# titus-leistner/mmlf

Hardware: AMD Instinct MI355X
Metric: 96x96 EPI patches/sec fwd+bwd, bs=512 (higher is better)
Workload: dtype f32 via 2 x f16 operand split (22 significant bits per operand, locally scaled; 3 MFMA passes, f32 accumulate)

## Files before the change

### mmlf_amd/csrc/wgrad.hip

```cpp
#include "conv_device.h"
#include "wgrad_map.h"

#ifdef MMLF_BOUNDS_DEBUG
int mmlf_oob_counts_wgrad(unsigned long long *host8, int reset)
{
    if (hipMemcpyFromSymbol(host8, HIP_SYMBOL(g_mmlf_oob), sizeof(unsigned long long) * 8) != hipSuccess) return 1;
    if (reset) {
        const unsigned long long z[8] = {};
        if (hipMemcpyToSymbol(HIP_SYMBOL(g_mmlf_oob), z, sizeof(z)) != hipSuccess) return 1;
    }
    return 0;
}
#endif

struct WgradArgs {
    const float *in;
    const float *g;
    float *part;
    long long NQpad;
    int cs_in, cin, cs_g, g_shift, P, nsplit, nslice, chunks_per_split, nchunks;
    int items;
    int g_cols;
    const float *in_amax, *g_amax;
    const float *chunk_scales;
// ... 150 lines not shown
__device__ __forceinline__ void split_store4(float4 v, char *p0, int plane_stride_bytes)
{
    unsigned h0, m0, l0, h1, m1, l1;
    split3_pair(v.x, v.y, h0, m0, l0);
    split3_pair(v.z, v.w, h1, m1, l1);
    *reinterpret_cast<uint2 *>(p0) = make_uint2(h0, h1);
    *reinterpret_cast<uint2 *>(p0 + plane_stride_bytes) = make_uint2(m0, m1);
    *reinterpret_cast<uint2 *>(p0 + 2 * plane_stride_bytes) = make_uint2(l0, l1);
}

template <int PL>
__device__ __forceinline__ void split_store4_pl(float4 v, float scale, char *p0, int plane_stride_bytes)
{
    if constexpr (PL == 3) {
        split_store4(v, p0, plane_stride_bytes);
    } else {
        unsigned h0, l0, h1, l1;
        split2_pair_f16<true>(v.x, v.y, scale, h0, l0);
        split2_pair_f16<true>(v.z, v.w, scale, h1, l1);
        *reinterpret_cast<uint2 *>(p0) = make_uint2(h0, h1);
        *reinterpret_cast<uint2 *>(p0 + plane_stride_bytes) = make_uint2(l0, l1);
    }
}
template <int PL>
__device__ __forceinline__ f32x4 mfma16_pl(bf16x8 x, bf16x8 y, f32x4 c)
{
    if constexpr (PL == 3) return __builtin_amdgcn_mfma_f32_16x16x32_bf16(x, y, c, 0, 0, 0);
    else return __builtin_amdgcn_mfma_f32_16x16x32_f16(__builtin_bit_cast(f16x8, x), __builtin_bit_cast(f16x8, y), c, 0, 0, 0);
}
template <int PL> __device__ __forceinline__ constexpr int term_a(int t)
{
    return PL == 3 ? (t == 0 ? 2 : t == 1 ? 0 : t <= 3 ? 1 : 0) : (t == 0 ? 1 : 0);
}
template <int PL> __device__ __forceinline__ constexpr int term_b(int t)
{
    return PL == 3 ? (t == 0 ? 0 : t == 1 ? 2 : t == 2 ? 1 : t == 3 ? 0 : t == 4 ? 1 : 0) : (t == 1 ? 1 : 0);
}
struct WgradScales { float inv_sa, inv_sg; };
template <int PL> __device__ __forceinline__ WgradScales wgrad_scales(const WgradArgs &a)
{
    WgradScales s = {1.f, 1.f};
    if constexpr (PL == 2) {
        s.inv_sa = a.chunk_scales[2 * (size_t)a.nchunks];
        s.inv_sg = a.chunk_scales[2 * (size_t)a.nchunks + 1];
    }
    return s;
}
template <int PL> __device__ __forceinline__ void wgrad_chunk_scale(const WgradArgs &a, int c, float &sa, float &sg)
{
    if constexpr (PL == 2) {
        const float2 v = *reinterpret_cast<const float2 *>(a.chunk_scales + 2 * (size_t)c);
        sa = __uint_as_float(__builtin_amdgcn_readfirstlane(__float_as_uint(v.x)));
        sg = __uint_as_float(__builtin_amdgcn_readfirstlane(__float_as_uint(v.y)));
    } else {
        sa = 1.f; sg = 1.f;
    }
}
struct ChunkScaleArgs {
    const float *in_amax, *g_amax;
    float *out;
    long long NQ;
    int nchunks, P, g_shift, nrows;
    Magic divP;
};
__device__ __forceinline__ int pow2_exponent(float p) { return (int)(__float_as_uint(p) >> 23) - 127; }
__global__ __launch_bounds__(256) void wgrad_chunk_scales_kernel(ChunkScaleArgs a)
{
    const int c = blockIdx.x * 256 + threadIdx.x;
    const float sA = pow2_scale_for(mmlf_amax_tensor_max(a.in_amax)), sG = pow2_scale_for(mmlf_amax_tensor_max(a.g_amax));
    if (c == 0) {
        a.out[2 * (size_t)a.nchunks] = 1.f / sA;
        a.out[2 * (size_t)a.nchunks + 1] = 1.f / sG;
    }
    if (c >= a.nchunks) return;
    const long long q0 = (long long)c * WG_KQ;
    int x = 0;
    if (q0 < a.NQ) {
        const long long ql = q0 + WG_KQ - 1;
        const unsigned r0 = fastdiv((unsigned)q0, a.divP);
        unsigned r1 = fastdiv((unsigned)(ql + a.P + 1), a.divP);
        if (r1 >= (unsigned)a.nrows) r1 = a.nrows - 1;
        float ma = 0.f, mg = 0.f;
        for (unsigned r = r0; r <= r1; ++r) ma = fmaxf(ma, a.in_amax[MMLF_AMAX_HEAD + r]);
        const unsigned g0 = fastdiv((unsigned)(q0 + a.g_shift), a.divP);
        unsigned g1 = fastdiv((unsigned)(ql + a.g_shift), a.divP);
        if (g1 >= (unsigned)a.nrows) g1 = a.nrows - 1;
        for (unsigned r = g0; r <= g1; ++r) mg = fmaxf(mg, a.g_amax[MMLF_AMAX_HEAD + r]);
        const int u = ma > 0.f ? pow2_exponent(pow2_scale_for(ma)) - pow2_exponent(sA) : 60;
        const int v = mg > 0.f ? pow2_exponent(pow2_scale_for(mg)) - pow2_exponent(sG) : 60;
        const int uu = u < 0 ? 0 : u, vv = v < 0 ? 0 : v;
        x = (uu - vv) >> 1;
        x = x > 15 ? 15 : (x < -24 ? -24 : x);
    }
    a.out[2 * (size_t)c] = sA * exp2f((float)x);
    a.out[2 * (size_t)c + 1] = sG * exp2f((float)-x);
}

template <int MB, int NB, int PL>
__global__ __launch_bounds__(256, 2) void wgrad4tap_x6n_kernel(WgradArgs a)
{
    constexpr int ROWA = 32 * (MB | 1), ROWG = 32 * (NB | 1);
    constexpr int A_PLANE = 34 * ROWA;
    constexpr int A_BYTES = 2 * PL * A_PLANE;
    constexpr int NTERM = PL == 3 ? 6 : 3;
    const WgradScales sc = wgrad_scales<PL>(a);
    constexpr int G_PLANE = WG_KQ * ROWG;
    constexpr int FA = 4 * MB, FG = 4 * NB;
    constexpr int NA = (66 * FA + 255) / 256, NG = (WG_KQ * FG + 255) / 256;
    constexpr bool HOLD_G = NB <= 5;
    extern __shared__ __attribute__((aligned(16))) char smem[];
    char *As = smem;
    char *Gs = smem + A_BYTES;

    const int tid = threadIdx.x;
    const int lane = tid & 63, t = tid >> 6;
    const int r16 = lane & 15, q4 = lane >> 4;
    int slice, split;
    if (!wgrad_block_map(blockIdx.x, a.nslice, a.nsplit, slice, split)) return;
    const int ci0 = slice * 16 * MB;
    int c_begin = split * a.chunks_per_split;
    int c_end = c_begin + a.chunks_per_split;
    if (c_end > a.nchunks) c_end = a.nchunks;

    f32x4 acc[MB][NB];
#pragma unroll
    for (int mb = 0; mb < MB; ++mb)
#pragma unroll
        for (int nb = 0; nb < NB; ++nb)
#pragma unroll
            for (int r = 0; r < 4; ++r) acc[mb][nb][r] = 0.f;

    float4 ra[NA], rg[NG];
#define WN_GLOAD(c)                                                                                         \
    do {                                                                                                    \
        const long long Qc = (long long)(c) * WG_KQ;                                                        \
        _Pragma("unroll") for (int j = 0; j < NA; ++j) {                                                    \
            const int idx = min(tid + 256 * j, 66 * FA - 1);                                                \
            const int row = idx / FA, f = idx - row * FA;                                                   \
            const int seg = row >= 33, pix = row - 33 * seg;                                                \
            const int ch = min(ci0 + 4 * f, a.cs_in - 4);                                                   \
            MMLF_OOB(OOB_WG_IN, ((Qc + seg * a.P + pix) * a.cs_in + ch + 4) * 4ll > a.in_bytes);            \
            ra[j] = *reinterpret_cast<const float4 *>(a.in + (size_t)(Qc + seg * a.P + pix) * a.cs_in + ch); \
        }                                                                                                   \
        _Pragma("unroll") for (int j = 0; j < NG; ++j) {                                                    \
            const int idx = min(tid + 256 * j, WG_KQ * FG - 1);                                             \
            const int row = idx / FG, f = idx - row * FG;                                                   \
            const int gc = min(4 * f, a.g_cols - 4);                                                        \
            MMLF_OOB(OOB_WG_G, ((Qc + a.g_shift + row) * a.cs_g + gc + 4) * 4ll > a.g_bytes);               \
            rg[j] = *reinterpret_cast<const float4 *>(a.g + (size_t)(Qc + a.g_shift + row) * a.cs_g + gc);  \
        }                                                                                                   \
    } while (0)
#define WN_LSTORE()                                                                                         \
    do {                                                                                                    \
        _Pragma("unroll") for (int j = 0; j < NA; ++j) {                                                    \
            const int idx = min(tid + 256 * j, 66 * FA - 1);                                                \
            const int row = idx / FA, f = idx - row * FA;                                                   \
            const int seg = row >= 33, pix = row - 33 * seg;                                                \
            float4 v = ra[j];                \
            const int ch = ci0 + 4 * f;      \
            if (ch == a.cin) v.x = sc.inv_sa;                                        \
            if (ch + 1 == a.cin) v.y = sc.inv_sa;                                                           \
            if (ch + 2 == a.cin) v.z = sc.inv_sa;                                                           \
            if (ch + 3 == a.cin) v.w = sc.inv_sa;                                                           \
            split_store4_pl<PL>(v, st_sa, As + seg * PL * A_PLANE + pix * ROWA + 8 * f, A_PLANE);           \
        }                                                                                                   \
        _Pragma("unroll") for (int j = 0; j < NG; ++j) {                                                    \
            const int idx = min(tid + 256 * j, WG_KQ * FG - 1);                                             \
            const int row = idx / FG, f = idx - row * FG;                                                   \
            split_store4_pl<PL>(rg[j], st_sg, Gs + row * ROWG + 8 * f, G_PLANE);                            \
        }                                                                                                   \
    } while (0)
    const int tq = (lane & 15) >> 2, tp = lane & 3;
    const char *a_lane = As + (t >> 1) * PL * A_PLANE + ((t & 1) + 4 * q4 + tq) * ROWA + 8 * tp;
    const char *g_lane = Gs + (4 * q4 + tq) * ROWG + 8 * tp;

    float st_sa = 1.f, st_sg = 1.f;
    if (c_begin < c_end) {
        WN_GLOAD(c_begin);
        for (int c = c_begin; c < c_end; ++c) {
            wgrad_chunk_scale<PL>(a, c, st_sa, st_sg);
            WN_LSTORE();
            __syncthreads();
            if (c + 1 < c_end) WN_GLOAD(c + 1);
            if constexpr (HOLD_G) {
                bf16x8 gf[NB][PL];
#pragma unroll
                for (int nb = 0; nb < NB; ++nb)
#pragma unroll
                    for (int pl = 0; pl < PL; ++pl) gf[nb][pl] = tr_frag(g_lane + pl * G_PLANE + 32 * nb, 4 * ROWG);
#pragma unroll
                for (int mb = 0; mb < MB; ++mb) {
                    bf16x8 af[PL];
#pragma unroll
                    for (int pl = 0; pl < PL; ++pl) af[pl] = tr_frag(a_lane + pl * A_PLANE + 32 * mb, 4 * ROWA);
#pragma unroll
                    for (int term = 0; term < NTERM; ++term)
#pragma unroll
                        for (int nb = 0; nb < NB; ++nb)
                            acc[mb][nb] = mfma16_pl<PL>(af[term_a<PL>(term)], gf[nb][term_b<PL>(term)], acc[mb][nb]);
                }
            } else {
                bf16x8 af[MB][PL];
#pragma unroll
                for (int mb = 0; mb < MB; ++mb)
#pragma unroll
                    for (int pl = 0; pl < PL; ++pl) af[mb][pl] = tr_frag(a_lane + pl * A_PLANE + 32 * mb, 4 * ROWA);
#pragma unroll
                for (int nb = 0; nb < NB; ++nb) {
                    bf16x8 gf[PL];
#pragma unroll
                    for (int pl = 0; pl < PL; ++pl) gf[pl] = tr_frag(g_lane + pl * G_PLANE + 32 * nb, 4 * ROWG);
#pragma unroll
                    for (int term = 0; term < NTERM; ++term)
#pragma unroll
                        for (int mb = 0; mb < MB; ++mb)
                            acc[mb][nb] = mfma16_pl<PL>(af[mb][term_a<PL>(term)], gf[term_b<PL>(term)], acc[mb][nb]);
                }
            }
            __syncthreads();
        }
    }
#undef WN_GLOAD
#undef WN_LSTORE
    constexpr int NP = 16 * NB;
    const int CIP = a.nslice * 16 * MB;
    float *pp = a.part + ((size_t)(split * 4 + t) * CIP + ci0) * NP;
#pragma unroll
    for (int mb = 0; mb < MB; ++mb)
#pragma unroll
        for (int nb = 0; nb < NB; ++nb)
#pragma unroll
            for (int r = 0; r < 4; ++r) {
                const int row = 16 * mb + 4 * q4 + r;
                const float un = (ci0 + row == a.cin ? 1.f : sc.inv_sa) * sc.inv_sg;
                MMLF_OOB(OOB_WG_PART, (long long)(pp - a.part) + (long long)row * NP + 16 * nb + r16 >= a.part_floats);
                pp[(size_t)row * NP + 16 * nb + r16] = acc[mb][nb][r] * un;
            }
}

template <int MB, int NBH, int PL>
__global__ __launch_bounds__(512, 2) void wgrad4tap_x6w_kernel(WgradArgs a)
{
    constexpr int NB = 2 * NBH;
    const WgradScales sc = wgrad_scales<PL>(a);
    constexpr int ROWA = 32 * (MB | 1), ROWG = 32 * (NB | 1);
    constexpr int A_PLANE = 34 * ROWA;
    constexpr int A_BYTES = 2 * PL * A_PLANE;
    constexpr int G_PLANE = WG_KQ * ROWG;
    constexpr int BUF_BYTES = A_BYTES + PL * G_PLANE;
    constexpr int FA = 4 * MB, FG = 4 * NB;
    constexpr int NA = (66 * FA + 511) / 512, NG = (WG_KQ * FG + 511) / 512;
    static_assert(2 * BUF_BYTES <= 160 * 1024, "LDS");
    extern __shared__ __attribute__((aligned(16))) char smem[];

    const int tid = threadIdx.x;
    const int lane = tid & 63;
    const int w = __builtin_amdgcn_readfirstlane(tid >> 6);
    const int t = w & 3, h = w >> 2;
    const int q4 = lane >> 4;

    float4 ra[NA], rg[NG];

    unsigned ga_off[NA], gg_off[NG];
    int la_off[NA], lg_off[NG], a_ch[NA];
#pragma unroll
    for (int j = 0; j < NA; ++j) {
        const int idx = min(tid + 512 * j, 66 * FA - 1);
        const int row = idx / FA, f = idx - row * FA;
        const int seg = row >= 33, pix = row - 33 * seg;
        la_off[j] = seg * PL * A_PLANE + pix * ROWA + 8 * f;
    }
#pragma unroll
    for (int j = 0; j < NG; ++j) {
        const int idx = min(tid + 512 * j, WG_KQ * FG - 1);
        const int row = idx / FG, f = idx - row * FG;
        gg_off[j] = (unsigned)((a.g_shift + row) * a.cs_g + min(4 * f, a.g_cols - 4)) * 4u;
        lg_off[j] = A_BYTES + row * ROWG + 8 * f;
    }
    const char *const in_b = reinterpret_cast<const char *>(a.in), *const g_b = reinterpret_cast<const char *>(a.g);
#define WW_GLOAD_A(j, c)                                                                                    \
    do {                                                                                                    \
        const long long cb_ = (long long)(c) * WG_KQ * a.cs_in * 4;                         \
        MMLF_OOB(OOB_WG_IN, cb_ + ga_off[j] + 16 > a.in_bytes);                                             \
         \
         \
        const __amdgpu_buffer_rsrc_t rs_ = __builtin_amdgcn_make_buffer_rsrc(                               \
            const_cast<char *>(in_b + cb_), 0, mmlf_records_left(a.in_bytes, cb_), MMLF_BUF_FLAGS);         \
        ra[j] = __builtin_bit_cast(float4, __builtin_amdgcn_raw_buffer_load_b128(rs_, ga_off[j], 0, 0));    \
    } while (0)
#define WW_GLOAD_G(j, c)                                                                                    \
// ... 187 lines not shown
    constexpr int U = 16;
    double acc[U];
#pragma unroll
    for (int u = 0; u < U; ++u) acc[u] = 0.0;
    int sp = 0;
    for (; sp + U <= nsplit; sp += U) {
        float v[U];
#pragma unroll
        for (int u = 0; u < U; ++u) v[u] = pp[(size_t)(sp + u) * stride];
#pragma unroll
        for (int u = 0; u < U; ++u) acc[u] += v[u];
    }
    for (; sp < nsplit; ++sp) acc[0] += pp[(size_t)sp * stride];
#pragma unroll
    for (int h = U / 2; h > 0; h >>= 1)
#pragma unroll
        for (int u = 0; u < h; ++u) acc[u] += acc[u + h];
    const double s = acc[0];
    if (ci == Cin) {
        gb[co] = accumulate ? gb[co] + (float)s : (float)s;
    } else {
        const size_t o = ((size_t)co * Cin + ci) * NTAP + master_tap<(NTAP == 4 ? 2 : 3)>(t, variant);
        gw[o] = accumulate ? gw[o] + (float)s : (float)s;
    }
}

__global__ __launch_bounds__(256) void wgrad_reduce_wave_kernel(const float *__restrict__ part, float *__restrict__ gw,
                                                                float *__restrict__ gb, int Cin, int Cout, int CIP, int NP,
                                                                int nsplit, int variant, int accumulate)
{
    const int total = 4 * (Cin + 1) * Cout;
    const int idx = blockIdx.x * 4 + (threadIdx.x >> 6), lane = threadIdx.x & 63;
    if (idx >= total) return;
    const int co = idx % Cout;
    int r = idx / Cout;
    const int ci = r % (Cin + 1);
    const int t = r / (Cin + 1);
    if (ci == Cin && (t != 0 || gb == nullptr)) return;
    const float *pp = part + ((size_t)t * CIP + ci) * NP + co;
    const size_t stride = (size_t)4 * CIP * NP;
    double acc = 0.0;
    for (int sp = lane; sp < nsplit; sp += 64) acc += pp[(size_t)sp * stride];
#pragma unroll
    for (int o = 32; o > 0; o >>= 1) acc += __shfl_xor(acc, o);
    if (lane) return;
    if (ci == Cin) {
        gb[co] = accumulate ? gb[co] + (float)acc : (float)acc;
    } else {
        const size_t o = ((size_t)co * Cin + ci) * 4 + master_tap<2>(t, variant);
        gw[o] = accumulate ? gw[o] + (float)acc : (float)acc;
    }
}

static int wgrad_nsplit(int nslice)
{
    int n = 512 / nslice;
    n = n / 8 * 8;
    if (n < 8) n = 8;
    return n;
}

struct Wgrad16Cfg { int mb, nb, nslice, nsplit; };
static inline bool wgrad16_cfg(int Cin, int Cout, long long nchunks, Wgrad16Cfg *c)
{
    if (Cout <= 0 || Cout > 288) return false;
    c->nb = Cout <= 32 ? 2 : Cout <= 80 ? 5 : Cout <= 128 ? 8 : 18;
    if (c->nb == 18) {
        c->mb = 3;
        wgrad_wide_splits(Cin, nchunks, device_cus(), c->nslice, c->nsplit);
    } else {
        c->mb = (c->nb <= 5 && Cin + 1 > 32 && Cin + 1 <= 80) ? 5 : 2;
        if (c->nb == 8 && Cin + 1 >= 128) c->mb = 3;
        c->nslice = (Cin + 1 + 16 * c->mb - 1) / (16 * c->mb);
        c->nsplit = wgrad_nsplit(c->nslice);
    }
    return true;
}

constexpr int WGRAD_MAX_COUT = 288, WGRAD_MAX_COUT_WIDE = 512;
static inline int wgrad_col_blocks(int Cout) { return Cout > WGRAD_MAX_COUT ? 2 : 1; }
static inline int wgrad_block_cout(int Cout, int b) { return b == 0 ? (Cout < WGRAD_MAX_COUT ? Cout : WGRAD_MAX_COUT) : Cout - WGRAD_MAX_COUT; }

struct WgradBlock {
    int c0, cout;
    int nt;
    Wgrad16Cfg cfg;
    int nslice, nsplit;
    int CIP, NP;
    int64_t part_floats;
};
struct WgradPlan {
    int nblocks;
    WgradBlock blk[2];
    int64_t part_floats;
    int64_t scales_off;
};
static bool wgrad_f32_block(int ks, int Cin, int c0, int cout, WgradBlock &k)
{
    k = {};
    k.c0 = c0; k.cout = cout; k.nt = pick_nt(cout);
    if (k.nt < 0) return false;
    const int ci_slices = (Cin + 1 + 31) / 32;
    k.nslice = (ks == 2 ? WgradF32Shape<2>::BPS : WgradF32Shape<3>::BPS) * ci_slices;
    k.nsplit = wgrad_nsplit(k.nslice);
    k.CIP = ci_slices * 32; k.NP = k.nt * 32;
    k.part_floats = (int64_t)k.nsplit * ks * ks * k.CIP * k.NP;
    return true;
}
static void wgrad_split_block(const Wgrad16Cfg &c, WgradBlock &k)
{
    k.nt = 0; k.cfg = c; k.nslice = c.nslice; k.nsplit = c.nsplit;
    k.CIP = c.nslice * 16 * c.mb; k.NP = 16 * c.nb;
    k.part_floats = (int64_t)k.nsplit * 4 * k.CIP * k.NP;
}
static bool wgrad_plan(int planes, int Cin, int Cout, long long nchunks, WgradPlan &p)
{
    p = {};
    if (Cout > WGRAD_MAX_COUT_WIDE) return false;
    p.nblocks = wgrad_col_blocks(Cout);
    for (int b = 0, c0 = 0; b < p.nblocks; c0 += p.blk[b++].cout) {
        WgradBlock &k = p.blk[b];
        WgradBlock largest = {};
        Wgrad16Cfg c;
        if (!wgrad_f32_block(2, Cin, c0, wgrad_block_cout(Cout, b), k)) return false;
        int64_t sized = k.part_floats;
        if (wgrad16_cfg(Cin, k.cout, -1, &c)) {
            wgrad_split_block(c, largest);
            if (largest.part_floats > sized) sized = largest.part_floats;
        }
        sized = (sized + 3) / 4 * 4;
        if (sized > p.scales_off) p.scales_off = sized;
        if (planes && wgrad16_cfg(Cin, k.cout, nchunks, &c)) wgrad_split_block(c, k);
        if (k.part_floats > p.part_floats) p.part_floats = k.part_floats;
    }
    return true;
}

extern "C" int64_t mmlf_wgrad_workspace_floats(int Cin, int Cout, int B, int H, int W)
{
    WgradPlan p;
    if (!wgrad_plan(0, Cin, Cout, -1, p) || B <= 0 || H <= 0 || W <= 0) return -1;
    return p.scales_off + 2 * (make_grid(B, H, W).NQpad / WG_KQ) + 4;
}

template <int KS, int NT>
static int launch_wgrad_f32(const WgradArgs &a, hipStream_t st)
{
    using S = WgradF32Shape<KS>;
    const dim3 grid(wgrad_grid_blocks(a.nslice, a.nsplit)), block(64 * S::WAVES);
    if constexpr (KS == 2) hipLaunchKernelGGL(wgrad4tap_kernel<NT>, grid, block, S::lds_bytes(NT), st, a);
    else hipLaunchKernelGGL(wgrad9tap_kernel<NT>, grid, block, S::lds_bytes(NT), st, a);
    return mmlf_launch_status(KS == 2 ? "mmlf_conv2x2_wgrad" : "mmlf_conv3x3_wgrad");
}

template <int MB, int NB, int PL>
static int launch_wgrad16(const WgradArgs &a, hipStream_t st)
{
    constexpr size_t lds = 2 * PL * 34 * 32 * (MB | 1) + PL * WG_KQ * 32 * (NB | 1);
    static PerDeviceOnce attr_once;
    if (attr_once.run([] { return mmlf_allow_lds(reinterpret_cast<const void *>(wgrad4tap_x6n_kernel<MB, NB, PL>), lds, "mmlf_conv2x2_wgrad_split"); }))
        return 1;
    hipLaunchKernelGGL((wgrad4tap_x6n_kernel<MB, NB, PL>), dim3(wgrad_grid_blocks(a.nslice, a.nsplit)), dim3(256), lds, st, a);
    return mmlf_launch_status("mmlf_conv2x2_wgrad_split");
}

static bool wgrad_persist()
{
    static const bool on = [] { const char *e = getenv("MMLF_WGRAD_PERSIST"); return !e || atoi(e) != 0; }();
    return on;
}

template <int PL>
static int launch_wgrad_wide(const WgradArgs &a, hipStream_t st)
{
    constexpr size_t lds = 2 * (2 * PL * 34 * 32 * (3 | 1) + PL * WG_KQ * 32 * (18 | 1));
    static PerDeviceOnce attr_once;
    if (attr_once.run([] { return mmlf_allow_lds(reinterpret_cast<const void *>(wgrad4tap_x6w_kernel<3, 9, PL>), lds, "mmlf_conv2x2_wgrad_split(wide)"); }))
        return 1;
    hipLaunchKernelGGL((wgrad4tap_x6w_kernel<3, 9, PL>), dim3(wgrad_wide_grid(a.items, device_cus(), wgrad_persist())), dim3(512), lds, st, a);
    return mmlf_launch_status("mmlf_conv2x2_wgrad_split");
}

template <int PL>
static int launch_wgrad_split(const Wgrad16Cfg &c, const WgradArgs &a, hipStream_t st)
{
    switch (10 * c.mb + c.nb) {
    case 22: return launch_wgrad16<2, 2, PL>(a, st);
    case 52: return launch_wgrad16<5, 2, PL>(a, st);
    case 25: return launch_wgrad16<2, 5, PL>(a, st);
    case 55: return launch_wgrad16<5, 5, PL>(a, st);
    case 28: return launch_wgrad16<2, 8, PL>(a, st);
    case 38: return launch_wgrad16<3, 8, PL>(a, st);
    default: return launch_wgrad_wide<PL>(a, st);
    }
}

static WgradArgs wgrad_args(const float *in, int cs_in, int Cin, const float *g, int cs_g, int g_shift, float *workspace,
                            const Grid &gr, long long alloc, long long part_floats)
{
    WgradArgs a = {};
    a.in = in; a.g = g; a.part = workspace; a.NQpad = gr.NQpad;
    a.cs_in = cs_in; a.cin = Cin; a.cs_g = a.g_cols = cs_g; a.g_shift = g_shift; a.P = gr.P;
    a.in_bytes = alloc * cs_in * 4; a.g_bytes = alloc * cs_g * 4;
    a.part_floats = part_floats;
    a.nchunks = (int)(gr.NQpad / WG_KQ);
    return a;
}
static void wgrad_set_grid(WgradArgs &a, int nslice, int nsplit)
{
    a.nslice = nslice;
    a.nsplit = nsplit;
    a.chunks_per_split = (a.nchunks + nsplit - 1) / nsplit;
    a.items = (int)wgrad_grid_blocks(nslice, nsplit);
}

template <int KS>
static int wgrad_reduce(const WgradArgs &a, float *gw, float *gb, int Cin, int Cout, int CIP, int NP, int variant,
                        int accumulate, hipStream_t st)
{
    const int total = KS * KS * (Cin + 1) * Cout;
    hipLaunchKernelGGL(wgrad_reduce_kernel<KS * KS>, dim3((total + 255) / 256), dim3(256), 0, st, a.part, gw, gb, Cin, Cout,
                       CIP, NP, a.nsplit, variant, accumulate);
// ... 252 lines not shown
```

### mmlf_amd/csrc/wgrad_map.h

```cpp
#pragma once

__host__ __device__ __forceinline__ bool wgrad_block_map(int b, int nslice, int nsplit, int &slice, int &split)
{
    const int x = b & 7, j = b >> 3;
    const int reg = (nsplit >> 3) * nslice;
    if (j < reg) {
        slice = j % nslice;
        split = (j / nslice) * 8 + x;
        return true;
    }
    const int left = (nsplit & 7) * nslice, per = (left + 7) >> 3;
    const int m = x * per + (j - reg);
    slice = m % nslice;
    split = (nsplit & ~7) + m / nslice;
    return m < left;
}

static inline unsigned wgrad_grid_blocks(int nslice, int nsplit)
{
    return 8u * (unsigned)((nsplit >> 3) * nslice + ((nsplit & 7) * nslice + 7) / 8);
}

static inline void wgrad_wide_splits(int Cin, long long nchunks, int cus, int &nslice, int &nsplit)
{
    nslice = (Cin + 1 + 47) / 48;
    if (cus > 256 || nchunks < 0) cus = 256;
    const int one_round = cus / nslice, three_rounds = (768 / nslice + 7) / 8 * 8;
    nsplit = nchunks < 0 ? (one_round > three_rounds ? one_round : three_rounds)
                         : (nchunks >= 42 * 1024 ? three_rounds : one_round);
    if (nsplit < 8) nsplit = 8;
}

static inline unsigned wgrad_wide_grid(int items, int cus, bool persist)
{
    if (!persist) return (unsigned)items;
    int resident = cus / 8 * 8;
    if (resident < 8) resident = 8;
    return (unsigned)(items < resident ? items : resident);
}
```

### mmlf_amd/engine.py

```python
import ctypes
import os
import threading

import torch

from . import _lib
from ._lib import call, check, ptr

VAR_IDENTITY, VAR_TRANSPOSE, VAR_TRANSPOSE_FLIPH = 0, 1, 2
BN_BLOCKS = 1024
LOSS_BLOCKS = 1024


MAX_WIDTH = {2: 512, 3: 288}
MAX_OC = 288
MAX_OVERLAP_WIDTH = 288


def cs_of(c):
    return (c + 7) // 8 * 8


class Geometry:

# ... 138 lines not shown
CONV_MODE = os.environ.get('MMLF_CONV_MODE', 'f16x3')
_PACK = {'f16x3': ('mmlf_packed_filter_h2_bytes', 1, 'mmlf_pack_filter_h2'),
         'bf16x6': ('mmlf_packed_filter_split_bytes', 1, 'mmlf_pack_filter_split'),
         'f32': ('mmlf_packed_filter_floats', 4, 'mmlf_pack_filter')}
_PACK3 = ('mmlf_packed_filter3x3_floats', 4, 'mmlf_pack_filter3x3')


def _pack(who, query, unit, entry, w, variant, dgrad):
    cout, cin = w.shape[0], w.shape[1]
    K, N = (cout, cin) if dgrad else (cin, cout)
    n = int(getattr(_lib.load(), query)(cs_of(K), N))
    if n < 0:
        raise RuntimeError(f'{who}: unsupported channels K={K} N={N}')
    out = torch.empty(n * unit // 4, dtype=torch.float32, device=w.device)
    call(entry, ptr(w), ptr(out), cout, cin, variant, int(dgrad), _lib.stream_ptr())
    return out


def pack_filter(w, variant, dgrad):
    return _pack('pack_filter', *_PACK.get(CONV_MODE, _PACK['f32']), w, variant, dgrad)


PROFILE = None


def _tic():
    e0, e1 = torch.cuda.Event(enable_timing=True), torch.cuda.Event(enable_timing=True)
    e0.record()
    return e0, e1


def _toc(events, tag, flops, nbytes):
    events[1].record()
    PROFILE.append((tag, flops, events[0], events[1], nbytes))


def _amax_of(geo, t, cs):
    a = getattr(t, 'absmax', None)
    if a is None:
        return geo.amax_of(t, cs)
    if CHECK_ABSMAX:
        true = geo.amax_of(t, cs)
        c = geo.amax_canonical(a)
        exact = geo.P >= 32
        bad = (c != true) if exact else (c < true)
        bad[0] = c[0] != true[0]
        if bool(bad.any()):
            k = int(bad.nonzero()[0])
            raise AssertionError(f'amax entry {k} holds {float(c[k])!r}, true max |x| is {float(true[k])!r}')
    return a


CHECK_ABSMAX = bool(os.environ.get('MMLF_CHECK_ABSMAX'))
OVERLAP_WGRAD = os.environ.get('MMLF_OVERLAP_WGRAD', '1') not in ('', '0')


CHECK_EXTENTS = bool(os.environ.get('MMLF_CHECK_EXTENTS'))
EXTENT_CHECKS = 0


def _audit(entry, scalars, n_ends, kind, have):
    global EXTENT_CHECKS
    ends = (ctypes.c_int64 * n_ends)()
    call(entry, *scalars, ends)
    for name, (k, t, off) in have.items():
        if t is None:
            continue
        got = t.untyped_storage().nbytes() - t.storage_offset() * t.element_size() - 4 * off
        if ends[k] > got:
            raise RuntimeError(f'MMLF_CHECK_EXTENTS: {kind}: the launch may touch {ends[k]} bytes behind `{name}`, '
                               f'the tensor has {got}')
    EXTENT_CHECKS += 1


def relu_bwd_slice(geo, src, cs_src, c_off, ref, cs_ref, ref_off, C, dst, cs_dst):
    amax = getattr(dst, 'absmax', None)
    if CHECK_EXTENTS:
        _audit('mmlf_audit_relu_bwd_slice', (cs_src, c_off, cs_ref, ref_off, C, cs_dst, geo.B, geo.H, geo.W), 4,
               f'relu_bwd_slice C={C} {cs_src}+{c_off} B={geo.B} {geo.H}x{geo.W}',
               {'src': (0, src, 0), 'ref': (1, ref, 0), 'dst': (2, dst, 0), 'amax': (3, amax, 0)})
    call('mmlf_relu_bwd_slice', ptr(src), cs_src, c_off, ptr(ref), cs_ref, ref_off, C, ptr(dst), cs_dst, geo.B, geo.H, geo.W,
         ptr(amax), _lib.stream_ptr())


THIN_MAX_N, THIN_MIN_K = 2, 64


def wgrad(geo, x, cs_in, cin, g, cs_g, cout, g_shift, gw, gb, variant, workspace, side=False):
    if cout <= THIN_MAX_N and cin >= THIN_MIN_K and cs_in <= 512:
        ws = _Workspace.get(x.device).scratch('thin_wgrad_side' if side else 'thin_wgrad', int(_lib.load().mmlf_conv2x2_wgrad_thin_workspace_floats(cin)))
        call('mmlf_conv2x2_wgrad_thin', ptr(x), cs_in, cin, ptr(g), cs_g, cout, g_shift, ptr(gw), ptr(gb), variant, 1,
             ptr(ws), geo.B, geo.H, geo.W, _lib.stream_ptr())
        return
    args = (ptr(x), cs_in, cin, ptr(g), cs_g, cout, g_shift, ptr(gw), ptr(gb), variant, 1, ptr(workspace),
            geo.B, geo.H, geo.W)
    prof = PROFILE is not None and cin >= 256 and cout >= 256
    if prof:
        events = _tic()
    if CONV_MODE == 'f16x3':
        ax, ag = _amax_of(geo, x, cs_in), _amax_of(geo, g, cs_g)
        if CHECK_EXTENTS:
            _audit('mmlf_audit_wgrad_h2', (cs_in, cin, cs_g, cout, g_shift, geo.B, geo.H, geo.W), 7,
                   f'wgrad {cin}->{cout} B={geo.B} {geo.H}x{geo.W} g_shift={g_shift}',
                   {'in': (0, x, 0), 'g': (1, g, 0), 'gw': (2, gw, 0), 'gb': (3, gb, 0), 'workspace': (4, workspace, 0),
                    'in_amax': (5, ax, 0), 'g_amax': (6, ag, 0)})
        call('mmlf_conv2x2_wgrad_h2', *args, ptr(ax), ptr(ag), _lib.stream_ptr())
    else:
# ... 291 lines not shown
            dev = stacks[0].device
            for name, t in zip('hvid', stacks):
                check(t, f'{name}_views', dev, shape=shape)
        self.check_params(p, dev)
        if packed is None:
            geo = Geometry(B, H, W, self.ksize)
        _Workspace.get(dev).enter_stream()
        fold = self.batchnorm and not train and (not save or (bool(frozen) and self.ksize == 2))
        relu_only = not self.batchnorm or fold
        packs = self._prepack(p, dev, save, input_grads, fold)
        tracked = []
        tape = {'geo': geo, 'device': dev, 'streams': [], 'out': [], 'packs': packs}
        if packed is not None:
            concat, xs = geo.buf(4 * self.chs, dev), list(xs_in)
        else:
            concat, *xs = geo.bufs([4 * self.chs] + [cs_of(cin0)] * 3, dev)
            xs.append(geo.buf(cs_of(cin0), dev))
        deferred = [] if (not fold and self.chs % 2 == 0 and all(b[-1].bn for _, _, b in self.streams)) else None
        for s, (key, var, blocks) in enumerate(self.streams):
            x = xs[s]
            if packed is None:
                call('mmlf_pack_nchw', ptr(stacks[s]), cin0, ptr(x), cs_of(cin0), B, H, W, ptr(x.absmax), _lib.stream_ptr())
            cs_x = cs_of(cin0)
            recs = []
            x_relu, xmask = False, None
            for k, spec in enumerate(blocks):
                last = k == len(blocks) - 1
                x, cs_x, xmask = self._block_fwd(geo, spec, var, x, cs_x, x_relu, xmask, p, train, recs if save else None,
                                                 out=concat if last else None, cs_out=4 * self.chs, c_off=s * self.chs,
                                                 packs=packs, tracked=tracked, deferred=deferred if last else None, fold=fold)
                x_relu = relu_only
            tape['streams'].append(recs)
        if deferred:
            arr = lambda k: (ctypes.c_void_p * 4)(*[ptr(d[k]) for d in deferred])
            call('mmlf_bn_apply_relu4', arr(0), cs_of(self.chs), self.chs, arr(1), arr(2), ptr(concat), 4 * self.chs,
                 B, H, W, ptr(concat.absmax), _lib.stream_ptr())
            del deferred[:]
        if save and relu_only:
            tape['concat'] = concat
        x, cs_x, x_relu, xmask = concat, 4 * self.chs, False, None
        for spec in self.out_blocks:
            x, cs_x, xmask = self._block_fwd(geo, spec, VAR_IDENTITY, x, cs_x, x_relu, xmask, p, train,
                                             tape['out'] if save else None, packs=packs, tracked=tracked, fold=fold)
            x_relu = relu_only
        if tracked:
            counts = {}
            for t in tracked:
                counts.setdefault(t.data_ptr(), [t, 0])[1] += 1
            torch._foreach_add_([t for t, _ in counts.values()], [n for _, n in counts.values()])
        out = torch.empty((B, self.oc, H, W), dtype=torch.float32, device=dev)
        call('mmlf_unpack_nchw', ptr(x), cs_x, ptr(out), self.oc, B, H, W, _lib.stream_ptr())
        return out, (tape if save else None)

    def _block_bwd(self, geo, rec, p, grads, gy, cs_gy, c_off, need_dx, after_bn=None, overlap=False, packs=None):
        spec, var = rec.spec, rec.var
        dev = gy.device
        ws = _Workspace.get(dev)
        B, H, W = geo.B, geo.H, geo.W
        C, cs_mid = spec.cout, cs_of(spec.cout)
        x, cs_x, y, z = rec.x, rec.cs_x, rec.y, rec.z
        pre = spec.prefix
        sp = _lib.stream_ptr
        packs = packs or {}
        f16 = CONV_MODE == 'f16x3' and self.ksize == 2
        bn = rec.bn
        assert grads is None or rec.pk2d is None, 'a frozen forward (BatchNorm folded) has no parameter gradients'
        if grads is not None:
            gw1, gb1, gw2, gb2 = (grads[f'{pre}.{k}'] for k in ('0.weight', '0.bias', '2.weight', '2.bias'))

        y_relu = {'mask_in': rec.ymask} if rec.ymask is not None and f16 else {'ref': y, 'cs_ref': cs_mid}
        x_relu = {}
        if rec.x_relu:
            x_relu = {'mask_in': rec.xmask} if rec.xmask is not None and f16 else {'ref': x, 'cs_ref': cs_x}

        got = geo.bufs(([cs_mid] if bn else []) + [cs_mid] + ([cs_x] if need_dx else []), dev)
        dy = got[1 if bn else 0]
        dx = got[-1] if need_dx else None
        if bn:
            if grads is None and rec.eval:
                coef = torch.zeros(3 * C, dtype=torch.float32, device=dev)
                coef[:C].copy_(rec.scale)
            else:
                coef = torch.empty(3 * C, dtype=torch.float32, device=dev)
                if grads is None:
                    dgb = ws.scratch('bn_dgamma_dbeta', 2 * C)
                    dgamma, dbeta, acc = dgb[:C], dgb[C:2 * C], 0
                else:
                    dgamma, dbeta, acc = grads[f'{pre}.3.weight'], grads[f'{pre}.3.bias'], 1
                call('mmlf_bn_bwd_reduce', ptr(gy), cs_gy, c_off, ptr(z), cs_mid, C, ptr(rec.scale), ptr(rec.shift),
                     ptr(p[f'{pre}.3.weight']), ptr(rec.smean), ptr(rec.sinv), ptr(dgamma), ptr(dbeta), acc, ptr(coef),
                     ptr(ws.partial), BN_BLOCKS, B, H, W, sp())
                if rec.eval:
                    coef[C:].zero_()
            dz = got[0]
            call('mmlf_bn_bwd_apply', ptr(gy), cs_gy, c_off, ptr(z), cs_mid, C, ptr(rec.scale), ptr(rec.shift),
                 ptr(rec.smean), ptr(coef), ptr(dz), cs_mid, B, H, W, ptr(dz.absmax), sp())
        else:
            assert c_off == 0 and cs_gy == cs_mid
            dz = gy
        if after_bn:
            after_bn()
        if grads is not None:
            self._wgrad(geo, True, y, cs_mid, C, dz, cs_mid, C, gw2, gb2, var)
        pk2d = rec.pk2d if rec.pk2d is not None else self._packed(packs, p, f'{pre}.2.weight', var, True)
        self._dgrad(geo, True, dz, cs_mid, C, pk2d, C, dy, cs_mid, **y_relu)
        del dz, got
        if overlap and need_dx and grads is not None:
            self._dgrad(geo, False, dy, cs_mid, C, self._packed(packs, p, f'{pre}.0.weight', var, True), spec.cin, dx, cs_x,
                        **x_relu)
            main = torch.cuda.current_stream()
            ready = main.record_event()
            with torch.cuda.stream(ws.side):
                ws.side.wait_event(ready)
                self._wgrad(geo, False, x, cs_x, spec.cin, dy, cs_mid, C, gw1, gb1, var, side=True)
                done = ws.side.record_event()
            return dx, done, (x, dy)
        if grads is not None:
            self._wgrad(geo, False, x, cs_x, spec.cin, dy, cs_mid, C, gw1, gb1, var)
        if need_dx:
            self._dgrad(geo, False, dy, cs_mid, C, self._packed(packs, p, f'{pre}.0.weight', var, True), spec.cin, dx, cs_x,
                        **x_relu)
        return dx, None, None

    def backward(self, p, tape, grad_output, grads, on_done=None, input_grads=None):
        geo, dev = tape['geo'], tape['device']
        check(grad_output, 'grad_output', dev, shape=(geo.B, self.oc, geo.H, geo.W), contiguous=False)
        if grads is not None:
            self._check_dict('grads', grads, self._grad_names, dev)
        _Workspace.get(dev).enter_stream()
        B, H, W = geo.B, geo.H, geo.W
        cs = cs_of(self.oc)
        g = geo.buf(cs, dev)
        call('mmlf_pack_nchw', ptr(grad_output.contiguous()), self.oc, ptr(g), cs, B, H, W, ptr(g.absmax),
             _lib.stream_ptr())
        cs_g = cs
        want = [bool(w) for w in input_grads] if input_grads is not None else [False] * 4
        assert len(want) == 4
        dstacks = [None] * 4
        recs = tape['out']
        main = torch.cuda.current_stream()
        pending = None

        def settle():
            nonlocal pending
            if pending is not None:
                main.wait_event(pending[0])
                if on_done:
                    on_done(pending[1])
                pending = None

        while recs:
            rec = recs.pop()
            wide = OVERLAP_WGRAD and 128 <= rec.spec.cin <= MAX_OVERLAP_WIDTH and self.ksize == 2
            g, event, keep = self._block_bwd(geo, rec, p, grads, g, cs_g, 0, True, after_bn=settle, overlap=wide,
                                             packs=tape['packs'])
            settle()
            if event is not None:
                pending = (event, rec.spec.prefix, keep)
            elif on_done:
                on_done(rec.spec.prefix)
            cs_g = rec.cs_x
        for s in reversed(range(4)):
            recs = tape['streams'][s]
            if s == 2:
                settle()
            gs, cs_s, off = g, cs_g, s * self.chs
            if 'concat' in tape:
                cs_s, off = cs_of(self.chs), 0
                gs = geo.buf(cs_s, dev)
                relu_bwd_slice(geo, g, cs_g, s * self.chs, tape['concat'], cs_g, s * self.chs, self.chs, gs, cs_s)
            while recs:
                rec = recs.pop()
                gs, _, _ = self._block_bwd(geo, rec, p, grads, gs, cs_s, off, need_dx=bool(recs) or want[s],
                                           packs=tape['packs'])
                cs_s, off = rec.cs_x, 0
            if want[s]:
                dstacks[s] = torch.empty((B, self.views, 3, H, W), dtype=torch.float32, device=dev)
                call('mmlf_unpack_nchw', ptr(gs), cs_s, ptr(dstacks[s]), 3 * self.views, B, H, W, _lib.stream_ptr())
            if on_done and s in (2, 0):
                on_done('in_net_id' if s == 2 else 'in_net_hv')
        return dstacks
```

Before: 1155.

## Overlap narrow-stream wgrad on side stream and make narrow wgrad kernel persistent

Narrow per-view streams now issue both wgrad GEMMs of each block on a side stream after the dgrads, so weight-gradient work overlaps the next block's backward on the main stream, with settle points before concatenation outputs. The wgrad16 kernel becomes a grid-stride persistent loop for NB==5, launching only about two blocks per CU. Per-thread global and LDS offsets are precomputed once per work item, and chunk scales are read through constant address space. This cuts address arithmetic and launch tail, at the cost of extra registers, keeping more tensors alive, and cross-stream contention.

```diff
diff --git a/mmlf_amd/csrc/wgrad.hip b/mmlf_amd/csrc/wgrad.hip
--- a/mmlf_amd/csrc/wgrad.hip
+++ b/mmlf_amd/csrc/wgrad.hip
@@ -226,6 +226,16 @@
         const float2 v = *reinterpret_cast<const float2 *>(a.chunk_scales + 2 * (size_t)c);
         sa = __uint_as_float(__builtin_amdgcn_readfirstlane(__float_as_uint(v.x)));
         sg = __uint_as_float(__builtin_amdgcn_readfirstlane(__float_as_uint(v.y)));
+    } else {
+        sa = 1.f; sg = 1.f;
+    }
+}
+template <int PL> __device__ __forceinline__ void wgrad_chunk_scale_const(const WgradArgs &a, int c, float &sa, float &sg)
+{
+    if constexpr (PL == 2) {
+        typedef const __attribute__((address_space(4))) float *cptr_t;
+        const cptr_t p = (cptr_t)(unsigned long long)(a.chunk_scales + 2 * (size_t)c);
+        sa = p[0]; sg = p[1];
     } else {
         sa = 1.f; sg = 1.f;
     }
@@ -286,73 +296,80 @@
     char *As = smem;
     char *Gs = smem + A_BYTES;
 
-    const int tid = threadIdx.x;
-    const int lane = tid & 63, t = tid >> 6;
-    const int r16 = lane & 15, q4 = lane >> 4;
-    int slice, split;
-    if (!wgrad_block_map(blockIdx.x, a.nslice, a.nsplit, slice, split)) return;
-    const int ci0 = slice * 16 * MB;
-    int c_begin = split * a.chunks_per_split;
-    int c_end = c_begin + a.chunks_per_split;
-    if (c_end > a.nchunks) c_end = a.nchunks;
-
-    f32x4 acc[MB][NB];
-#pragma unroll
-    for (int mb = 0; mb < MB; ++mb)
-#pragma unroll
-        for (int nb = 0; nb < NB; ++nb)
-#pragma unroll
-            for (int r = 0; r < 4; ++r) acc[mb][nb][r] = 0.f;
+    const int t = __builtin_amdgcn_readfirstlane(threadIdx.x >> 6);
 
     float4 ra[NA], rg[NG];
+    unsigned ga_off[NA], gg_off[NG];
+    int la_off[NA], lg_off[NG], a_ch[NA];
+    const char *const in_b = reinterpret_cast<const char *>(a.in), *const g_b = reinterpret_cast<const char *>(a.g);
 #define WN_GLOAD(c)                                                                                         \
     do {                                                                                                    \
-        const long long Qc = (long long)(c) * WG_KQ;                                                        \
+        const long long ca_ = (long long)(c) * WG_KQ * a.cs_in * 4, cg_ = (long long)(c) * WG_KQ * a.cs_g * 4;    \
         _Pragma("unroll") for (int j = 0; j < NA; ++j) {                                                    \
-            const int idx = min(tid + 256 * j, 66 * FA - 1);                                                \
-            const int row = idx / FA, f = idx - row * FA;                                                   \
-            const int seg = row >= 33, pix = row - 33 * seg;                                                \
-            const int ch = min(ci0 + 4 * f, a.cs_in - 4);                                                   \
-            MMLF_OOB(OOB_WG_IN, ((Qc + seg * a.P + pix) * a.cs_in + ch + 4) * 4ll > a.in_bytes);            \
-            ra[j] = *reinterpret_cast<const float4 *>(a.in + (size_t)(Qc + seg * a.P + pix) * a.cs_in + ch); \
+            MMLF_OOB(OOB_WG_IN, ca_ + ga_off[j] + 16 > a.in_bytes);                                         \
+            ra[j] = *reinterpret_cast<const float4 *>(in_b + ca_ + ga_off[j]);                              \
         }                                                                                                   \
         _Pragma("unroll") for (int j = 0; j < NG; ++j) {                                                    \
-            const int idx = min(tid + 256 * j, WG_KQ * FG - 1);                                             \
-            const int row = idx / FG, f = idx - row * FG;                                                   \
-            const int gc = min(4 * f, a.g_cols - 4);                                                        \
-            MMLF_OOB(OOB_WG_G, ((Qc + a.g_shift + row) * a.cs_g + gc + 4) * 4ll > a.g_bytes);               \
-            rg[j] = *reinterpret_cast<const float4 *>(a.g + (size_t)(Qc + a.g_shift + row) * a.cs_g + gc);  \
+            MMLF_OOB(OOB_WG_G, cg_ + gg_off[j] + 16 > a.g_bytes);                                           \
+            rg[j] = *reinterpret_cast<const float4 *>(g_b + cg_ + gg_off[j]);                               \
         }                                                                                                   \
     } while (0)
 #define WN_LSTORE()                                                                                         \
     do {                                                                                                    \
         _Pragma("unroll") for (int j = 0; j < NA; ++j) {                                                    \
-            const int idx = min(tid + 256 * j, 66 * FA - 1);                                                \
-            const int row = idx / FA, f = idx - row * FA;                                                   \
-            const int seg = row >= 33, pix = row - 33 * seg;                                                \
             float4 v = ra[j];                \
-            const int ch = ci0 + 4 * f;      \
+            const int ch = a_ch[j];          \
             if (ch == a.cin) v.x = sc.inv_sa;                                        \
             if (ch + 1 == a.cin) v.y = sc.inv_sa;                                                           \
             if (ch + 2 == a.cin) v.z = sc.inv_sa;                                                           \
             if (ch + 3 == a.cin) v.w = sc.inv_sa;                                                           \
-            split_store4_pl<PL>(v, st_sa, As + seg * PL * A_PLANE + pix * ROWA + 8 * f, A_PLANE);           \
+            split_store4_pl<PL>(v, st_sa, As + la_off[j], A_PLANE);                                         \
         }                                                                                                   \
-        _Pragma("unroll") for (int j = 0; j < NG; ++j) {                                                    \
-            const int idx = min(tid + 256 * j, WG_KQ * FG - 1);                                             \
-            const int row = idx / FG, f = idx - row * FG;                                                   \
-            split_store4_pl<PL>(rg[j], st_sg, Gs + row * ROWG + 8 * f, G_PLANE);                            \
-        }                                                                                                   \
+        _Pragma("unroll") for (int j = 0; j < NG; ++j) split_store4_pl<PL>(rg[j], st_sg, Gs + lg_off[j], G_PLANE); \
     } while (0)
+    for (int b = blockIdx.x; b < a.items; b += gridDim.x) {
+    int slice, split;
+    if (!wgrad_block_map(b, a.nslice, a.nsplit, slice, split)) continue;
+    const int ci0 = slice * 16 * MB;
+    int c_begin = split * a.chunks_per_split;
+    int c_end = c_begin + a.chunks_per_split;
+    if (c_end > a.nchunks) c_end = a.nchunks;
+
+    f32x4 acc[MB][NB];
+#pragma unroll
+    for (int mb = 0; mb < MB; ++mb)
+#pragma unroll
+        for (int nb = 0; nb < NB; ++nb)
+#pragma unroll
+            for (int r = 0; r < 4; ++r) acc[mb][nb][r] = 0.f;
+    int lane;
+    asm volatile("v_mbcnt_lo_u32_b32 %0, -1, 0\n\tv_mbcnt_hi_u32_b32 %0, -1, %0" : "=v"(lane));
+    const int tid = lane + 64 * t;
+#pragma unroll
+    for (int j = 0; j < NA; ++j) {
+        const int idx = min(tid + 256 * j, 66 * FA - 1);
+        const int row = idx / FA, f = idx - row * FA;
+        const int seg = row >= 33, pix = row - 33 * seg;
+        la_off[j] = seg * PL * A_PLANE + pix * ROWA + 8 * f;
+        a_ch[j] = ci0 + 4 * f;
+        ga_off[j] = (unsigned)((seg * a.P + pix) * a.cs_in + min(ci0 + 4 * f, a.cs_in - 4)) * 4u;
+    }
+#pragma unroll
+    for (int j = 0; j < NG; ++j) {
+        const int idx = min(tid + 256 * j, WG_KQ * FG - 1);
+        const int row = idx / FG, f = idx - row * FG;
+        gg_off[j] = (unsigned)((a.g_shift + row) * a.cs_g + min(4 * f, a.g_cols - 4)) * 4u;
+        lg_off[j] = row * ROWG + 8 * f;
+    }
     const int tq = (lane & 15) >> 2, tp = lane & 3;
-    const char *a_lane = As + (t >> 1) * PL * A_PLANE + ((t & 1) + 4 * q4 + tq) * ROWA + 8 * tp;
-    const char *g_lane = Gs + (4 * q4 + tq) * ROWG + 8 * tp;
+    const char *a_lane = As + (t >> 1) * PL * A_PLANE + ((t & 1) + 4 * (lane >> 4) + tq) * ROWA + 8 * tp;
+    const char *g_lane = Gs + (4 * (lane >> 4) + tq) * ROWG + 8 * tp;
 
     float st_sa = 1.f, st_sg = 1.f;
     if (c_begin < c_end) {
         WN_GLOAD(c_begin);
         for (int c = c_begin; c < c_end; ++c) {
-            wgrad_chunk_scale<PL>(a, c, st_sa, st_sg);
+            wgrad_chunk_scale_const<PL>(a, c, st_sa, st_sg);
             WN_LSTORE();
             __syncthreads();
             if (c + 1 < c_end) WN_GLOAD(c + 1);
@@ -394,11 +411,12 @@
             __syncthreads();
         }
     }
-#undef WN_GLOAD
-#undef WN_LSTORE
     constexpr int NP = 16 * NB;
     const int CIP = a.nslice * 16 * MB;
     float *pp = a.part + ((size_t)(split * 4 + t) * CIP + ci0) * NP;
+    int lane_e;
+    asm volatile("v_mbcnt_lo_u32_b32 %0, -1, 0\n\tv_mbcnt_hi_u32_b32 %0, -1, %0" : "=v"(lane_e));
+    const int r16 = lane_e & 15, q4 = lane_e >> 4;
 #pragma unroll
     for (int mb = 0; mb < MB; ++mb)
 #pragma unroll
@@ -410,6 +428,9 @@
                 MMLF_OOB(OOB_WG_PART, (long long)(pp - a.part) + (long long)row * NP + 16 * nb + r16 >= a.part_floats);
                 pp[(size_t)row * NP + 16 * nb + r16] = acc[mb][nb][r] * un;
             }
+    }
+#undef WN_GLOAD
+#undef WN_LSTORE
 }
 
 template <int MB, int NBH, int PL>
@@ -703,14 +724,6 @@
     }
 }
 
-static int wgrad_nsplit(int nslice)
-{
-    int n = 512 / nslice;
-    n = n / 8 * 8;
-    if (n < 8) n = 8;
-    return n;
-}
-
 struct Wgrad16Cfg { int mb, nb, nslice, nsplit; };
 static inline bool wgrad16_cfg(int Cin, int Cout, long long nchunks, Wgrad16Cfg *c)
 {
@@ -720,7 +733,7 @@
         c->mb = 3;
         wgrad_wide_splits(Cin, nchunks, device_cus(), c->nslice, c->nsplit);
     } else {
-        c->mb = (c->nb <= 5 && Cin + 1 > 32 && Cin + 1 <= 80) ? 5 : 2;
+        c->mb = wgrad_narrow_mb(Cin, c->nb);
         if (c->nb == 8 && Cin + 1 >= 128) c->mb = 3;
         c->nslice = (Cin + 1 + 16 * c->mb - 1) / (16 * c->mb);
         c->nsplit = wgrad_nsplit(c->nslice);
@@ -804,6 +817,12 @@
     return mmlf_launch_status(KS == 2 ? "mmlf_conv2x2_wgrad" : "mmlf_conv3x3_wgrad");
 }
 
+static bool wgrad_persist()
+{
+    static const bool on = [] { const char *e = getenv("MMLF_WGRAD_PERSIST"); return !e || atoi(e) != 0; }();
+    return on;
+}
+
 template <int MB, int NB, int PL>
 static int launch_wgrad16(const WgradArgs &a, hipStream_t st)
 {
@@ -811,14 +830,9 @@
     static PerDeviceOnce attr_once;
     if (attr_once.run([] { return mmlf_allow_lds(reinterpret_cast<const void *>(wgrad4tap_x6n_kernel<MB, NB, PL>), lds, "mmlf_conv2x2_wgrad_split"); }))
         return 1;
-    hipLaunchKernelGGL((wgrad4tap_x6n_kernel<MB, NB, PL>), dim3(wgrad_grid_blocks(a.nslice, a.nsplit)), dim3(256), lds, st, a);
+    const unsigned grid = NB == 5 ? wgrad_narrow_grid(a.items, device_cus(), wgrad_persist()) : (unsigned)a.items;
+    hipLaunchKernelGGL((wgrad4tap_x6n_kernel<MB, NB, PL>), dim3(grid), dim3(256), lds, st, a);
     return mmlf_launch_status("mmlf_conv2x2_wgrad_split");
-}
-
-static bool wgrad_persist()
-{
-    static const bool on = [] { const char *e = getenv("MMLF_WGRAD_PERSIST"); return !e || atoi(e) != 0; }();
-    return on;
 }
 
 template <int PL>
diff --git a/mmlf_amd/csrc/wgrad_map.h b/mmlf_amd/csrc/wgrad_map.h
--- a/mmlf_amd/csrc/wgrad_map.h
+++ b/mmlf_amd/csrc/wgrad_map.h
@@ -38,3 +38,21 @@
     if (resident < 8) resident = 8;
     return (unsigned)(items < resident ? items : resident);
 }
+
+static inline int wgrad_nsplit(int nslice)
+{
+    int n = 512 / nslice;
+    n = n / 8 * 8;
+    if (n < 8) n = 8;
+    return n;
+}
+
+static inline int wgrad_narrow_mb(int Cin, int nb) { return (nb <= 5 && Cin + 1 > 32 && Cin + 1 <= 80) ? 5 : 2; }
+
+static inline unsigned wgrad_narrow_grid(int items, int cus, bool persist)
+{
+    if (!persist) return (unsigned)items;
+    int resident = 2 * (cus / 8 * 8);
+    if (resident < 16) resident = 16;
+    return (unsigned)(items < resident ? items : resident);
+}
diff --git a/mmlf_amd/engine.py b/mmlf_amd/engine.py
--- a/mmlf_amd/engine.py
+++ b/mmlf_amd/engine.py
@@ -214,7 +214,9 @@
 
 
 CHECK_ABSMAX = bool(os.environ.get('MMLF_CHECK_ABSMAX'))
-OVERLAP_WGRAD = os.environ.get('MMLF_OVERLAP_WGRAD', '1') not in ('', '0')
+OVERLAP_WGRAD = os.environ.get('MMLF_OVERLAP_WGRAD', '3') not in ('', '0')
+NARROW_OVERLAP = {'2': 1, '3': 2}.get(os.environ.get('MMLF_OVERLAP_WGRAD', '3'), 0)
+MAX_NARROW_OVERLAP_WIDTH = 80
 
 
 CHECK_EXTENTS = bool(os.environ.get('MMLF_CHECK_EXTENTS'))
@@ -612,7 +614,7 @@
         call('mmlf_unpack_nchw', ptr(x), cs_x, ptr(out), self.oc, B, H, W, _lib.stream_ptr())
         return out, (tape if save else None)
 
-    def _block_bwd(self, geo, rec, p, grads, gy, cs_gy, c_off, need_dx, after_bn=None, overlap=False, packs=None):
+    def _block_bwd(self, geo, rec, p, grads, gy, cs_gy, c_off, need_dx, after_bn=None, overlap=False, packs=None, narrow=0):
         spec, var = rec.spec, rec.var
         dev = gy.device
         ws = _Workspace.get(dev)
@@ -660,10 +662,23 @@
             dz = gy
         if after_bn:
             after_bn()
-        if grads is not None:
+        narrow = narrow if grads is not None else 0
+        if grads is not None and narrow < 2:
             self._wgrad(geo, True, y, cs_mid, C, dz, cs_mid, C, gw2, gb2, var)
         pk2d = rec.pk2d if rec.pk2d is not None else self._packed(packs, p, f'{pre}.2.weight', var, True)
         self._dgrad(geo, True, dz, cs_mid, C, pk2d, C, dy, cs_mid, **y_relu)
+        if narrow:
+            if need_dx:
+                self._dgrad(geo, False, dy, cs_mid, C, self._packed(packs, p, f'{pre}.0.weight', var, True), spec.cin, dx, cs_x,
+                            **x_relu)
+            ready = torch.cuda.current_stream().record_event()
+            with torch.cuda.stream(ws.side):
+                ws.side.wait_event(ready)
+                if narrow == 2:
+                    self._wgrad(geo, True, y, cs_mid, C, dz, cs_mid, C, gw2, gb2, var, side=True)
+                self._wgrad(geo, False, x, cs_x, spec.cin, dy, cs_mid, C, gw1, gb1, var, side=True)
+                done = ws.side.record_event()
+            return dx, done, (x, dy, y, dz) if narrow == 2 else (x, dy)
         del dz, got
         if overlap and need_dx and grads is not None:
             self._dgrad(geo, False, dy, cs_mid, C, self._packed(packs, p, f'{pre}.0.weight', var, True), spec.cin, dx, cs_x,
@@ -705,7 +720,7 @@
             nonlocal pending
             if pending is not None:
                 main.wait_event(pending[0])
-                if on_done:
+                if on_done and pending[1] is not None:
                     on_done(pending[1])
                 pending = None
 
@@ -720,9 +735,11 @@
             elif on_done:
                 on_done(rec.spec.prefix)
             cs_g = rec.cs_x
+        narrow = NARROW_OVERLAP if (OVERLAP_WGRAD and grads is not None and CONV_MODE == 'f16x3' and self.ksize == 2
+                                    and self.batchnorm and self.chs <= MAX_NARROW_OVERLAP_WIDTH) else 0
         for s in reversed(range(4)):
             recs = tape['streams'][s]
-            if s == 2:
+            if s == 2 and not narrow:
                 settle()
             gs, cs_s, off = g, cs_g, s * self.chs
             if 'concat' in tape:
@@ -731,12 +748,21 @@
                 relu_bwd_slice(geo, g, cs_g, s * self.chs, tape['concat'], cs_g, s * self.chs, self.chs, gs, cs_s)
             while recs:
                 rec = recs.pop()
-                gs, _, _ = self._block_bwd(geo, rec, p, grads, gs, cs_s, off, need_dx=bool(recs) or want[s],
-                                           packs=tape['packs'])
+                if narrow:
+                    gs, event, keep = self._block_bwd(geo, rec, p, grads, gs, cs_s, off, need_dx=bool(recs) or want[s],
+                                                      after_bn=settle, packs=tape['packs'],
+                                                      narrow=narrow if (recs or s) else 0)
+                    if event is not None:
+                        pending = (event, None, keep)
+                else:
+                    gs, _, _ = self._block_bwd(geo, rec, p, grads, gs, cs_s, off, need_dx=bool(recs) or want[s],
+                                               packs=tape['packs'])
                 cs_s, off = rec.cs_x, 0
             if want[s]:
                 dstacks[s] = torch.empty((B, self.views, 3, H, W), dtype=torch.float32, device=dev)
                 call('mmlf_unpack_nchw', ptr(gs), cs_s, ptr(dstacks[s]), 3 * self.views, B, H, W, _lib.stream_ptr())
             if on_done and s in (2, 0):
+                settle()
                 on_done('in_net_id' if s == 2 else 'in_net_hv')
+        settle()
         return dstacks
```

New measurement: 1159 (median of 5 runs). Within noise of the previous version (+0.3%).
